# encryptorion-lab/phantom-fhe

Hardware: AMD Instinct MI355X
Metric: forward NTT limb-transforms/s at N=2^16, 45 RNS moduli (higher is better)
Workload: dtype u64; 1 GPU; CKKS N=2^16, 45 data limbs (+15 special), forward NTT of a batch of 16 ciphertext polynomials per step (720 limb-transforms, 360 MiB, HBM-resident; configs[2] parameter set); N=65536, limbs=45, special_limbs=15, parallelism=ciphertext-batch x1, launch=K steps enqueued by one library call (2 K eager kernel launches)

## Files before the change

### phantom-fhe_amd/csrc/pha_ntt.hip

```cpp
#include "../../include/phantom_amd.h"
#include "pha_internal.h"
#include "pha_experiments.h"
#include "pha_ntt_core.h"

#include <atomic>
#include <type_traits>

namespace pha {

constexpr int kPassHoist = 0;
#ifndef PHA_NTT_PASS_ORDER
#define PHA_NTT_PASS_ORDER 1
#endif
#ifndef PHA_NTT_ORDER_INT_HEAD
#define PHA_NTT_ORDER_INT_HEAD 1
#endif
#if defined(PHA_EXPERIMENTS)
std::atomic<int> g_ntt_variant{kDefaultVariant};
static inline int ntt_variant() { return g_ntt_variant.load(std::memory_order_relaxed); }
std::atomic<int> g_whole14_min{1 << 30};
std::atomic<int> g_fused_split{0};
std::atomic<int> g_fused_lag{2};
std::atomic<int> g_fused_min_tiles{1 << 30};
extern std::atomic<int> g_bconv_split;
// ... 41 lines not shown
template <bool FWD, int EPI, bool FOLD>
__device__ __forceinline__ void tile_args(const NttKArgs &k, uint32_t twr, uint32_t tile, PassArgs &a) {
    const uint32_t prime = twr >= k.sel.remap_from ? twr + k.sel.remap_add : twr;
    const size_t n = (size_t)1 << k.log_n;
    a.in = k.in + (size_t)twr * n;
    a.out = k.out + (size_t)twr * n;
    a.tw = k.tw + (size_t)prime * n;
    a.twd = nullptr;
    a.q = k.mod[prime].value;
    a.tile = tile;
    a.rho0 = k.t1;
    a.stride = k.t2;
    if (!FWD && FOLD) {
        a.ninv = k.ninv[prime];
        a.w1ninv = k.w1ninv[prime];
    }
    a.pro_reduce = false;
    a.pro_ratio1 = 0;
    a.fp = false;
    if (k.fpinfo) {
        const FpInfo fi = k.fpinfo[prime];
        if (fi.ok) {
            a.fp = true;
            a.fpm = FpMod{fi.q, fi.qinv, (fi.ok & 2) != 0, (fi.ok & 4) != 0};
            a.twd = k.twf + (size_t)prime * n;
            if (!FWD && FOLD) {
                a.ninv = k.ninvf[prime];
                a.w1ninv = k.w1ninvf[prime];
            }
        }
    }
    if (EPI == EPI_INV_SCALE || EPI == EPI_FWD_MODDOWN || EPI == EPI_FWD_MODDOWN_ADD || EPI == EPI_FWD_KSRESCALE) {
        a.scale.x = k.scale[twr];
        a.scale.y = k.scale_shoup[twr];
    }
    a.aux = (EPI == EPI_FWD_MODDOWN || EPI == EPI_FWD_MODDOWN_ADD || EPI == EPI_FWD_KSRESCALE || EPI == EPI_INV_CANON_ADD) ? k.aux + (size_t)twr * n : nullptr;
    if (EPI == EPI_FWD_KSRESCALE) {
        a.scale2.x = k.scale2[twr];
        a.scale2.y = k.scale2_shoup[twr];
        a.aux2 = k.aux2 + (size_t)twr * n;
    }
}

PHA_HD bool limb_excluded(const NttKArgs &k, uint32_t twr, uint32_t z) {
    const uint32_t zd = k.excl_mod ? z % k.excl_mod : z;
    const uint32_t es = k.sel.excl_start + zd * k.excl_step;
    uint32_t ee = es + (k.sel.excl_end - k.sel.excl_start);
    ee = ee < k.excl_limit ? ee : k.excl_limit;
    return twr >= es && twr < ee;
}

template <class C, bool FWD, int EPI, bool FOLD>
__device__ __forceinline__ void full_tile_args(const NttKArgs &k, uint32_t twr, uint32_t z, uint32_t tile, PassArgs &a) {
    tile_args<FWD, EPI, FOLD>(k, twr, tile, a);
    if (k.batch > 1) {
        a.in += (size_t)z * k.in_stride;
        a.out += (size_t)z * k.out_stride;
        if (EPI == EPI_FWD_MODDOWN || EPI == EPI_FWD_MODDOWN_ADD || EPI == EPI_FWD_KSRESCALE) a.aux += (size_t)z * k.aux_stride;
        if (EPI == EPI_FWD_KSRESCALE) a.aux2 += (size_t)z * k.aux2_stride;
    }
    if (EPI == EPI_INV_CANON_ADD) a.aux += (size_t)(z >> 1) * k.aux_pair_stride + (size_t)(z & 1) * k.aux_stride;
    if (FWD && (C::STRIDED || C::WHOLE) && k.pro_src) {
        const uint32_t prime = twr >= k.sel.remap_from ? twr + k.sel.remap_add : twr;
        a.in = k.pro_src + (size_t)z * k.pro_stride;
        a.pro_reduce = true;
        a.pro_ratio1 = k.mod[prime].ratio1;
        a.pro_half = bfv_lift_threshold(k.pro_t);
        a.pro_inc = bfv_lift_increment(a.q, k.pro_t);
    }
}

template <class C, bool FWD, int EPI, bool FOLD, int HOIST, bool COH, int ONLY = 0, int PRO = PRO_NONE>
__device__ __forceinline__ void exec_pass(const PassArgs &a, u64 *lds, int tid) {
    u64 reg[C::EPT];
    u64x2 twreg[C::TW_TOTAL];
    using Prog = PassProgram<C, FWD, EPI, FOLD, HOIST, COH, PRO>;
    auto pass = [&](const PassArgs &pa) __attribute__((always_inline)) {
        Prog::load_twiddles(pa, tid, twreg);
        Prog::template run_pass<SEG_PLAIN, false>(pa, lds, tid, reg, twreg);
    };
    PHA_WITH_FP_KNOWN(a, ONLY != 2 && a.fp, pass);
}

template <class C, bool FWD, int EPI, bool FOLD>
__global__ __launch_bounds__(C::THREADS) void ntt_zloop_kernel(const NttKArgs k, const ZloopMap m) {
    static_assert(!C::WHOLE, "the batched form exists for the passes of the two-pass plans");
    extern __shared__ __attribute__((aligned(16))) unsigned char smem[];
    u64 *lds = reinterpret_cast<u64 *>(smem);
    __builtin_amdgcn_s_setprio(3);
    const int tid = threadIdx.x;
    uint32_t b = blockIdx.x;
    PassArgs a;
    if (b < m.int_blocks) {
        const uint32_t tile = b % m.tiles, rest = b / m.tiles, z = rest % k.batch, twr = k.sel.start + m.limb[rest / k.batch];
        if (limb_excluded(k, twr, z)) return;
        full_tile_args<C, FWD, EPI, FOLD>(k, twr, z, tile, a);
        exec_pass<C, FWD, EPI, FOLD, 0, false, 2>(a, lds, tid);
        return;
    }
    b -= m.int_blocks;
    const uint32_t tile = b % m.tiles, rest = b / m.tiles, zgroups = (k.batch + m.zper - 1) / m.zper;
    const uint32_t twr = k.sel.start + m.limb[m.n_int + rest / zgroups];
    const uint32_t z0 = (rest % zgroups) * m.zper, z1 = (z0 + m.zper < k.batch) ? z0 + m.zper : k.batch;
    full_tile_args<C, FWD, EPI, FOLD>(k, twr, z0, tile, a);
    using Prog = PassProgram<C, FWD, EPI, FOLD, 1, false>;
    a.fp = true;
    u64x2 twreg[C::TW_TOTAL];
    Prog::load_twiddles(a, tid, twreg);
    u64 regA[C::EPT], regB[C::EPT];
    auto args_of = [&](uint32_t z) __attribute__((always_inline)) {
        PassArgs b = a;
        const size_t dz = (size_t)(z - z0);
        b.in += dz * k.in_stride;
        b.out += dz * k.out_stride;
        if (EPI == EPI_FWD_MODDOWN || EPI == EPI_FWD_MODDOWN_ADD || EPI == EPI_FWD_KSRESCALE) b.aux += dz * k.aux_stride;
        if (EPI == EPI_FWD_KSRESCALE) b.aux2 += dz * k.aux2_stride;
        return b;
    };
    auto transform = [&](const PassArgs &b, u64 *reg) __attribute__((always_inline)) {
        Prog::template run_pass<SEG_PREFETCHED, true>(b, lds, tid, reg, twreg);
    };
    auto next = [&](uint32_t z) __attribute__((always_inline)) {
        while (z < z1 && limb_excluded(k, twr, z)) z++;
        return z;
    };
    uint32_t z = next(z0);
    if (z >= z1) return;
    Prog::prefetch(args_of(z), tid, regA);
    __builtin_amdgcn_s_setprio(0);
    for (;;) {
        uint32_t zn = next(z + 1);
        if (zn < z1) Prog::prefetch(args_of(zn), tid, regB);
        transform(args_of(z), regA);
        if (zn >= z1) break;
        z = zn;
        zn = next(z + 1);
        if (zn < z1) Prog::prefetch(args_of(zn), tid, regA);
        transform(args_of(z), regB);
        if (zn >= z1) break;
        z = zn;
    }
}

template <class C, bool FWD, int EPI, bool FOLD, int HOIST, int PRO = PRO_NONE>
__global__ __launch_bounds__(C::THREADS) void ntt_pass_kernel(const NttKArgs k, const PassOrder o) {
    extern __shared__ __attribute__((aligned(16))) unsigned char smem[];
    u64 *lds = reinterpret_cast<u64 *>(smem);

    __builtin_amdgcn_s_setprio(3);
    uint32_t tile = blockIdx.x, y = blockIdx.y, z = blockIdx.z;
    if (k.zfast_tiles) {
        const uint32_t b = blockIdx.x, per_chunk = k.zfast_run * k.batch, chunk = b / per_chunk, rem = b - chunk * per_chunk;
        z = rem / k.zfast_run;
        const uint32_t group = chunk * k.zfast_run + (rem - z * k.zfast_run);
        if (group >= k.zfast_tiles * k.sel.count) return;
        tile = group % k.zfast_tiles;
        y = group / k.zfast_tiles;
    }
#if PHA_NTT_PASS_ORDER
    else if (o.tiles) {
        if (!pass_order_decode(o, k.batch, blockIdx.x, blockIdx.y, blockIdx.z, y, z, tile)) return;
    }
#endif
    const uint32_t twr = k.sel.start + y;
    if (limb_excluded(k, twr, z)) return;
    PassArgs a;
    full_tile_args<C, FWD, EPI, FOLD>(k, twr, z, tile, a);
    exec_pass<C, FWD, EPI, FOLD, HOIST, false, 0, PRO>(a, lds, threadIdx.x);
}

static void raise_lds_limit(const void *kernel, size_t bytes, std::atomic<uint64_t> &raised) {
    if (bytes <= 64 * 1024) return;
    int dev = 0;
    PHA_HIP(hipGetDevice(&dev));
    const uint64_t bit = 1ull << (dev & 63);
    if (raised.load(std::memory_order_acquire) & bit) return;
    PHA_HIP(hipFuncSetAttribute(kernel, hipFuncAttributeMaxDynamicSharedMemorySize, (int)bytes));
    raised.fetch_or(bit, std::memory_order_release);
}

template <class C, bool FWD, int EPI, bool FOLD, int PRO = PRO_NONE>
static void launch_pass(const NttKArgs &k, hipStream_t s, const PassOrder *order = nullptr) {
    const size_t n = (size_t)1 << k.log_n;
    const size_t lds_bytes = (size_t)C::LDS_WORDS * sizeof(u64);
    const unsigned tiles_per_limb = (unsigned)(n >> C::LOGTILE);
    dim3 grid(tiles_per_limb, k.sel.count, k.batch);
    NttKArgs kk = k;
    kk.zfast_tiles = 0;
    if (!C::STRIDED && !C::WHOLE && k.zfast_tiles) {
        kk.zfast_tiles = tiles_per_limb;
        kk.zfast_run = 8;
        const unsigned groups = tiles_per_limb * k.sel.count;
        grid = dim3(((groups + kk.zfast_run - 1) / kk.zfast_run) * kk.zfast_run * k.batch, 1, 1);
    }
    PassOrder o{};
    if (order && !kk.zfast_tiles) {
        o = *order;
        pass_order_grid(o, k.batch, grid.x, grid.y, grid.z);
    }
    static std::atomic<uint64_t> raised{0};
    raise_lds_limit(reinterpret_cast<const void *>(&ntt_pass_kernel<C, FWD, EPI, FOLD, kPassHoist, PRO>), lds_bytes, raised);
    hipLaunchKernelGGL((ntt_pass_kernel<C, FWD, EPI, FOLD, kPassHoist, PRO>), grid, dim3(C::THREADS), lds_bytes, s, kk, o);
    check_launch();
}

#if defined(PHA_EXPERIMENTS)
}
#include "pha_ntt_onelaunch.h"
namespace pha {
constexpr bool kExperiments = true;
#else
constexpr bool kExperiments = false;
#endif

template <int E> using EpiC = std::integral_constant<int, E>;
template <int P> using ProC = std::integral_constant<int, P>;
template <bool FWD, class F>
static void dispatch_epi(int epi, F &&f) {
    if constexpr (FWD) {
        if (epi == EPI_FWD_MODDOWN) f(EpiC<EPI_FWD_MODDOWN>{});
        else if (epi == EPI_FWD_MODDOWN_ADD) f(EpiC<EPI_FWD_MODDOWN_ADD>{});
        else if (epi == EPI_FWD_KSRESCALE) f(EpiC<EPI_FWD_KSRESCALE>{});
        else f(EpiC<EPI_FWD_CANON>{});
    } else {
        if (epi == EPI_INV_SCALE) f(EpiC<EPI_INV_SCALE>{});
        else if (epi == EPI_INV_CANON_ADD) f(EpiC<EPI_INV_CANON_ADD>{});
        else f(EpiC<EPI_INV_CANON>{});
    }
}
template <class F>
static void dispatch_pro(const NttKArgs &k, F &&f) {
    if (k.pro_t) f(ProC<PRO_LIFT>{});
    else f(ProC<PRO_NONE>{});
}

template <class P>
static void launch_inverse_last(const NttKArgs &k, int epi, hipStream_t s, const PassOrder *order = nullptr) {
    dispatch_epi<false>(epi, [&](auto e) { launch_pass<P, false, e(), true>(k, s, order); });
}

template <class W, bool FWD>
static void launch_whole(NttKArgs k, int epi, hipStream_t s) {
    k.t1 = 1;
    k.t2 = W::T;
    k.mid = k.out;
    if constexpr (FWD) {
        dispatch_epi<true>(epi, [&](auto e) {
            if constexpr (e() == EPI_FWD_CANON) dispatch_pro(k, [&](auto p) { launch_pass<W, true, EPI_FWD_CANON, false, p()>(k, s); });
            else launch_pass<W, true, e(), false>(k, s);
        });
    } else {
        launch_inverse_last<W>(k, epi, s);
    }
}

template <class C>
static bool plan_zloop(const NttKArgs &k, ZloopMap &m) {
    if (k.pro_src || k.sel.count > 128) return false;
    uint8_t fp[128];
    for (uint32_t y = 0; y < k.sel.count; y++) {
        const uint32_t twr = k.sel.start + y, prime = twr >= k.sel.remap_from ? twr + k.sel.remap_add : twr;
        fp[y] = k.fpinfo != nullptr && (k.h_primes[prime] >> 50) == 0;
    }
    return zloop_plan(m, k.sel.count, fp, k.batch, (uint32_t)(((size_t)1 << k.log_n) >> C::LOGTILE), C::THREADS / 64, kZloopMinBatch);
}
template <class C, bool FWD, int EPI, bool FOLD>
static void launch_zloop(const NttKArgs &k, const ZloopMap &m, hipStream_t s) {
    NttKArgs kk = k;
    kk.zfast_tiles = 0;
    const size_t lds_bytes = (size_t)C::LDS_WORDS * sizeof(u64);
    hipLaunchKernelGGL((ntt_zloop_kernel<C, FWD, EPI, FOLD>), dim3(zloop_blocks(m, k.batch)), dim3(C::THREADS), lds_bytes, s, kk, m);
    check_launch();
}
template <class C>
static void launch_zloop_forward(const NttKArgs &k, const ZloopMap &m, int epi, hipStream_t s) {
    dispatch_epi<true>(epi, [&](auto e) { launch_zloop<C, true, e(), false>(k, m, s); });
}

constexpr size_t kLastLevelCacheBytes = (size_t)256 << 20;
static NttKArgs limb_range(const NttKArgs &k, uint32_t lo, uint32_t cnt) {
    NttKArgs h = k;
    h.sel.start = k.sel.start + lo;
    h.sel.count = cnt;
    return h;
}
static uint32_t order_parts(const NttKArgs &k) {
    const size_t bytes = ((size_t)k.sel.count * k.batch << k.log_n) * sizeof(u64);
    return PHA_NTT_PASS_ORDER == 2 && k.sel.count >= 2 && bytes > kLastLevelCacheBytes ? 2u : 1u;
}

template <class F>
static void for_each_order_part(const NttKArgs &k, const ZloopMap &m, int strided_logtile, F &&pair) {
    if (PHA_NTT_PASS_ORDER == 0) return pair(0u, k.sel.count, m, (const PassOrder *)nullptr);
    const uint32_t parts = order_parts(k), cut = pass_order_half(k.sel.count);
    for (uint32_t h = 0; h < parts; h++) {
        const uint32_t lo = h * cut, hi = parts == 1 ? k.sel.count : h ? k.sel.count : cut;
        const ZloopMap mh = parts == 1 ? m : zloop_sub(m, lo, hi, k.batch);
        const PassOrder o = pass_order_reverse(mh, (uint32_t)(((size_t)1 << k.log_n) >> strided_logtile), PHA_NTT_ORDER_INT_HEAD != 0);
        pair(lo, hi - lo, mh, &o);
    }
}

constexpr int kIpPlan = 3;
template <int LOGN, int VARIANT>
struct TwoPass {
    using P1 = typename NttPlan<LOGN, VARIANT>::P1;
    using P2 = typename NttPlan<LOGN, VARIANT>::P2;
    static constexpr bool ZLOOP = zloop_variant(VARIANT) >= 0;
    using Z2 = typename NttPlan<LOGN, ZLOOP ? zloop_variant(VARIANT) : VARIANT>::P2;
    static constexpr bool ONE_LAUNCH = kExperiments && P1::THREADS == 512 && P1::LOGTILE == 12 && P2::THREADS == 64;
    NttKArgs k1, k2;
    explicit TwoPass(NttKArgs k) {
        k.t1 = P1::T;
        k.t2 = P2::T;
        k1 = k2 = k;
        k1.out = k.mid;
        k1.out_stride = k.poly_stride;
        k2.in = k.mid;
        k2.in_stride = k.poly_stride;
    }
};

template <int LOGN, int VARIANT>
static void forward_impl(const NttKArgs &k_in, int epi, hipStream_t s, Context *fused) {
    using T = TwoPass<LOGN, VARIANT>;
    using P1 = typename T::P1;
    using P2 = typename T::P2;
    T t(k_in);
    const NttKArgs &k1 = t.k1;
    NttKArgs &k = t.k2;
    k.pro_src = nullptr;
    if (k.first_pass_done && !(LOGN == 16 && VARIANT == 10 && P1::LOGT == 6))
        throw std::logic_error("ntt_forward: first_pass_done needs the 64 x 1024 plan the fused conversion wrote");
#if defined(PHA_EXPERIMENTS)
    if constexpr (T::ONE_LAUNCH) {
        if (fused && epi != EPI_FWD_KSRESCALE && !k.first_pass_done && !k.pro_t) {
            bool done = false;
            dispatch_epi<true>(epi, [&](auto e) {
                if constexpr (e() != EPI_FWD_KSRESCALE) done = launch_fused<P1, P2, true, e(), false>(*fused, k1, k, s);
            });
            if (done) return;
        }
    }
#endif
    auto strided = [&](const NttKArgs &ka, const PassOrder *order) {
        dispatch_pro(ka, [&](auto p) { launch_pass<P1, true, EPI_NONE, false, p()>(ka, s, order); });
    };
    if constexpr (T::ZLOOP) {
        using Z2 = typename T::Z2;
        ZloopMap m;
        if (!k.first_pass_only && plan_zloop<Z2>(k, m)) {
            if (k.first_pass_done) return launch_zloop_forward<Z2>(k, m, epi, s);
            return for_each_order_part(k, m, P1::LOGTILE, [&](uint32_t lo, uint32_t cnt, const ZloopMap &mh, const PassOrder *o) {
// ... 401 lines not shown
```

### phantom-fhe_amd/csrc/pha_ntt_core.h

```cpp
#pragma once
#include "pha_arith.h"
#include "pha_bfv_lift.h"

namespace pha {

constexpr int kTileElems = 4096;

enum Epilogue {
    EPI_NONE = 0,
    EPI_FWD_CANON = 1,
    EPI_FWD_MODDOWN = 2,
    EPI_INV_CANON = 3,
    EPI_INV_SCALE = 4,
    EPI_FWD_MODDOWN_ADD = 5,
    EPI_FWD_KSRESCALE = 6,
    EPI_INV_CANON_ADD = 7,
};

enum Prologue {
    PRO_NONE = 0,
    PRO_LIFT = 1,
};

template <int LOGT_, bool STRIDED_, int R0_, int R1_, int R2_ = 0, int EPT_ = 16, bool OT_ = false, int LOGTILE_ = 12,
          bool WHOLE_ = false, int R3_ = 0>
struct PassCfg {
    static constexpr int EPT = EPT_;
    static constexpr bool OT = OT_ && !STRIDED_;
    static constexpr int LOGTILE = LOGTILE_;
    static constexpr int TILE = 1 << LOGTILE_;
    static constexpr int THREADS = TILE / EPT_;
    static_assert(LOGTILE_ >= LOGT_ && LOGTILE_ <= 14, "a tile holds whole transforms and fits the LDS budget (2^14 words + padding = 144 KiB of the 160 KiB)");
    static constexpr bool WAVE_LOCAL = TILE / EPT_ == 64;
    static constexpr bool WHOLE = WHOLE_ && !STRIDED_;
    static_assert((1 << R0_) <= EPT_ && (1 << R1_) <= EPT_ && (1 << R2_) <= EPT_ && (1 << R3_) <= EPT_, "radix exceeds registers");
    static_assert(!R3_ || R2_, "rounds are filled in order");
    static constexpr int LOGT = LOGT_;
    static constexpr int T = 1 << LOGT_;
    static constexpr int LOGV = LOGTILE_ - LOGT_;
    static constexpr int V = 1 << LOGV;
    static constexpr bool STRIDED = STRIDED_;
    static constexpr int NR = R3_ ? 4 : R2_ ? 3 : 2;
    static_assert(R0_ + R1_ + R2_ + R3_ == LOGT_, "round schedule must cover all stages");
    static_assert(LOGT_ >= 4 && LOGT_ <= 14, "tile transform length out of range");
    static_assert(THREADS >= 64, "a workgroup is at least one wavefront");
    static constexpr int r(int i) { return i == 0 ? R0_ : i == 1 ? R1_ : i == 2 ? R2_ : R3_; }
    static constexpr bool ot_round(int i) { return OT && i == NR - 1; }
    static constexpr int tw_count(int i) {
        return !r(i) ? 0 : ot_round(i) ? ((1 << r(i)) - 1) + (EPT_ >> r(i)) * r(i) : (EPT_ >> r(i)) * ((1 << r(i)) - 1);
    }
    static constexpr int tw_off(int i) {
        return i == 0 ? 0 : i == 1 ? tw_count(0) : i == 2 ? tw_count(0) + tw_count(1) : tw_count(0) + tw_count(1) + tw_count(2);
    }
    static constexpr int TW_TOTAL = tw_count(0) + tw_count(1) + tw_count(2) + tw_count(3);
    static constexpr int s0(int i) { return i == 0 ? 0 : i == 1 ? R0_ : i == 2 ? R0_ + R1_ : R0_ + R1_ + R2_; }
    static constexpr int PITCH = T + ((T >> 4) << 1);
    static constexpr int LDS_WORDS = STRIDED_ ? (T * V + (T >> 4) * 16) : (V * PITCH);
    static constexpr int lds_index(int e, int v) {
        return STRIDED_ ? (e * V + v + ((e >> 4) << 4)) : (v * PITCH + e + ((e >> 4) << 1));
    }
};

struct PassArgs {
    const u64 *in;
    u64 *out;
    const u64x2 *tw;
    const u64 *twd;
    u64 q;
    u32 tile;
    u32 rho0;
    u32 stride;
    u64x2 ninv, w1ninv;
    u64x2 scale;
    const u64 *aux;
    u64x2 scale2;
    const u64 *aux2;
    bool fp;
    FpMod fpm;
    bool pro_reduce;
    u64 pro_ratio1;
    u64 pro_half, pro_inc;
};

template <class C>
PHA_HD size_t global_index(const PassArgs &a, int e, int v) {
    if (C::STRIDED) return (size_t)e * a.stride + (size_t)a.tile * C::V + v;
    return ((size_t)a.tile * C::V + v) * C::T + e;
}

template <class C, int RI>
PHA_HD void decode_group(int g, int &v, int &hi, int &lo) {
    constexpr int r = C::r(RI), s0 = C::s0(RI), LOGD = C::LOGT - s0 - r;
    if (C::STRIDED) {
        v = g & (C::V - 1);
        int rest = g >> C::LOGV;
        lo = rest & ((1 << LOGD) - 1);
        hi = rest >> LOGD;
    } else {
        lo = g & ((1 << LOGD) - 1);
        int rest = g >> LOGD;
        hi = rest & ((1 << s0) - 1);
        v = rest >> s0;
    }
}

PHA_HD u64x2 tw_entry(const PassArgs &a, u32 idx) {
    if (a.fp) return u64x2{a.twd[idx], 0};
    return a.tw[idx];
}
template <int R>
PHA_HD void load_group_twiddles(u64x2 *t, const PassArgs &a, u32 base0) {
    if (a.fp) {
#pragma unroll
        for (int j = 0; j < R; j++)
#pragma unroll
            for (int kk = 0; kk < (1 << j); kk++) t[(1 << j) - 1 + kk].x = a.twd[(base0 << j) + kk];
        return;
    }
#pragma unroll
    for (int j = 0; j < R; j++)
#pragma unroll
        for (int kk = 0; kk < (1 << j); kk++) t[(1 << j) - 1 + kk] = a.tw[(base0 << j) + kk];
}

template <int R>
PHA_HD void ct_round(u64 *v, const u64x2 *t, u64 q4, u64 nq) {
#pragma unroll
    for (int j = 0; j < R; j++) {
        const int dist = 1 << (R - 1 - j);
#pragma unroll
        for (int k = 0; k < (1 << R); k++) {
            if (k & dist) continue;
            const int kk = k >> (R - j);
            ct_bfly4(v[k], v[k + dist], t[(1 << j) - 1 + kk], q4, nq);
        }
    }
}

template <int R, bool FWD>
PHA_HD void ot_round_int(u64 *v, const u64x2 *tc, const u64x2 *tr, u64 q4, u64 nq) {
#pragma unroll
    for (int jj = 0; jj < R; jj++) {
        const int j = FWD ? jj : R - 1 - jj;
        const int dist = 1 << (R - 1 - j);
#pragma unroll
        for (int k = 0; k < (1 << R); k++) {
            if (k & dist) continue;
// ... 187 lines not shown
    return *p;
}
template <bool NT>
PHA_HD void gstore(u64 *p, u64 v) {
#if defined(__HIP_DEVICE_COMPILE__)
    if (NT) {
        __builtin_nontemporal_store(v, p);
        return;
    }
#endif
    *p = v;
}
template <bool NT>
PHA_HD void gstore2(u64x2 *p, u64x2 v) {
#if defined(__HIP_DEVICE_COMPILE__)
    if (NT) {
        __builtin_nontemporal_store(u64v2{v.x, v.y}, reinterpret_cast<u64v2 *>(p));
        return;
    }
#endif
    *p = v;
}

template <class C, int RI, bool FROM_GLOBAL, bool COH = false>
PHA_HD void round_load(const PassArgs &a, const u64 *lds, int tid, u64 *reg) {
    constexpr int r = C::r(RI), K = 1 << r, G = C::EPT >> r, s0 = C::s0(RI);
    constexpr int LOGD = C::LOGT - s0 - r;
#pragma unroll
    for (int gi = 0; gi < G; gi++) {
        int v, hi, lo;
        decode_group<C, RI>(tid + C::THREADS * gi, v, hi, lo);
        u64 *rg = reg + gi * K;
        const int e0 = (hi << (LOGD + r)) + lo;
        if (FROM_GLOBAL && COH) {
#if defined(__HIP_DEVICE_COMPILE__)
            if constexpr (!C::STRIDED && K == 8 && G == 1 && LOGD >= 1 && LOGD <= 6) {
                const bool odd = lo & 1;
                const u64 *base = a.in + global_index<C>(a, e0 - (odd ? 1 : 0) + ((odd ? 4 : 0) << LOGD), v);
                u64x2 w0, w1, w2, w3;
                asm volatile("global_load_dwordx4 %0, %4, off sc1\n\t"
                             "global_load_dwordx4 %1, %4, off offset:%5 sc1\n\t"
                             "global_load_dwordx4 %2, %4, off offset:%6 sc1\n\t"
                             "global_load_dwordx4 %3, %4, off offset:%7 sc1\n\t"
                             "s_waitcnt vmcnt(0)"
                             : "=&v"(w0), "=&v"(w1), "=&v"(w2), "=&v"(w3)
                             : "v"(base), "n"(8 << LOGD), "n"(16 << LOGD), "n"(24 << LOGD)
                             : "memory");
                const u64x2 w[4] = {w0, w1, w2, w3};
#pragma unroll
                for (int j = 0; j < 4; j++) {
                    const u64 send = odd ? w[j].x : w[j].y;
                    const u32 slo = (u32)__builtin_amdgcn_update_dpp(0, (int)(u32)send, 0xB1, 0xF, 0xF, false);
                    const u32 shi = (u32)__builtin_amdgcn_update_dpp(0, (int)(u32)(send >> 32), 0xB1, 0xF, 0xF, false);
                    const u64 recv = ((u64)shi << 32) | slo;
                    rg[j] = odd ? recv : w[j].x;
                    rg[4 + j] = odd ? w[j].y : recv;
                }
                continue;
            }
#endif
#pragma unroll
            for (int k = 0; k < K; k++) rg[k] = coherent_load(a.in + global_index<C>(a, e0 + (k << LOGD), v));
        } else if (FROM_GLOBAL) {
            if (!C::STRIDED && LOGD == 0) {
                const u64x2 *p = reinterpret_cast<const u64x2 *>(a.in + global_index<C>(a, e0, v));
#pragma unroll
                for (int k = 0; k < K; k += 2) {
                    u64x2 t = gload2<false>(p + (k >> 1));
                    rg[k] = t.x;
                    rg[k + 1] = t.y;
                }
            } else {
#pragma unroll
                for (int k = 0; k < K; k++) rg[k] = gload<false>(a.in + global_index<C>(a, e0 + (k << LOGD), v));
            }
        } else {
#pragma unroll
            for (int k = 0; k < K; k++) rg[k] = lds[C::lds_index(e0 + (k << LOGD), v)];
        }
    }
}

template <class C, int RI>
PHA_HD void round_load_tw(const PassArgs &a, int tid, u64x2 *twreg) {
    constexpr int r = C::r(RI), K = 1 << r, G = C::EPT >> r, s0 = C::s0(RI);
    if (C::ot_round(RI)) {
        static_assert(!C::ot_round(RI) || (C::THREADS % (1 << s0)) == 0, "groups of a thread must share hi");
        u64x2 *base = twreg + C::tw_off(RI);
        int v, hi, lo;
        decode_group<C, RI>(tid, v, hi, lo);
        load_group_twiddles<r>(base, a, (u32)hi);
#pragma unroll
        for (int gi = 0; gi < G; gi++) {
            decode_group<C, RI>(tid + C::THREADS * gi, v, hi, lo);
            const u32 rho = a.rho0 + a.tile * C::V + (u32)v;
#pragma unroll
            for (int j = 0; j < r; j++) base[(K - 1) + gi * r + j] = tw_entry(a, rho << (s0 + j));
        }
        return;
    }
#pragma unroll
    for (int gi = 0; gi < G; gi++) {
        int v, hi, lo;
        decode_group<C, RI>(tid + C::THREADS * gi, v, hi, lo);
        const u32 rho = C::STRIDED ? 1u : (a.rho0 + a.tile * C::V + (u32)v);
        const u32 base0 = (rho << s0) + (u32)hi;
        load_group_twiddles<r>(twreg + C::tw_off(RI) + gi * (K - 1), a, base0);
    }
}

template <class C, int RI, bool FWD, bool FOLD, bool RECENTRE = false, bool GSFULL = false>
PHA_HD void round_compute(const PassArgs &a, int tid, u64 *reg, const u64x2 *twreg) {
    constexpr int r = C::r(RI), K = 1 << r, G = C::EPT >> r;
    const u64 q4 = a.q << 2, nq = 0 - a.q;
    if (C::ot_round(RI)) {
        const u64x2 *tc = twreg + C::tw_off(RI);
#pragma unroll
        for (int gi = 0; gi < G; gi++) {
            u64 *rg = reg + gi * K;
            const u64x2 *tr = tc + (K - 1) + gi * r;
            if (a.fp) {
                if (FWD ? a.fpm.ct_light : a.fpm.gs_light) ot_round_fp<r, FWD, true>(rg, tc, tr, a.fpm);
                else ot_round_fp<r, FWD, false>(rg, tc, tr, a.fpm);
            } else {
                ot_round_int<r, FWD>(rg, tc, tr, q4, nq);
            }
        }
        return;
    }
    if (a.fp) {
#pragma unroll
        for (int gi = 0; gi < G; gi++) {
            u64 *rg = reg + gi * K;
            const u64x2 *t = twreg + C::tw_off(RI) + gi * (K - 1);
            if (FWD) {
                fp_ct_round<r>(rg, t, a.fpm);
                if (RECENTRE && !a.fpm.ct_light) {
#pragma unroll
                    for (int k = 0; k < K; k++) rg[k] = as_u64(fp_reduce(as_f64(rg[k]), a.fpm));
                }
            } else if (a.fpm.gs_light) {
                constexpr int stage0 = C::LOGT - C::s0(RI) - r;
                constexpr bool canon_in = !C::STRIDED;
                const bool light = C::LOGT <= 9 || a.fpm.q < (double)(1ull << (52 - C::LOGT));
                if (light) fp_gs_round<r, FOLD, true>(rg, t, a.fpm, a.ninv, a.w1ninv);
                else fp_gs_round<r, FOLD, false, stage0, canon_in>(rg, t, a.fpm, a.ninv, a.w1ninv);
            } else {
                if (GSFULL) {
                    constexpr bool canon = RI == C::NR - 1 && (!C::STRIDED || C::WHOLE);
                    fp_gs_round<r, FOLD, false, 0, canon>(rg, t, a.fpm, a.ninv, a.w1ninv);
                } else {
                    fp_gs_round<r, FOLD, true>(rg, t, a.fpm, a.ninv, a.w1ninv);
                }
                if (RECENTRE) {
#pragma unroll
                    for (int k = 0; k < K; k++) rg[k] = as_u64(fp_reduce(as_f64(rg[k]), a.fpm));
                }
            }
        }
        return;
    }
#pragma unroll
    for (int gi = 0; gi < G; gi++) {
        u64 *rg = reg + gi * K;
        const u64x2 *t = twreg + C::tw_off(RI) + gi * (K - 1);
        if (FWD) ct_round<r>(rg, t, q4, nq);
        else gs_round<r, FOLD>(rg, t, q4, nq, a.ninv, a.w1ninv);
    }
}

template <class C, int RI, bool TO_GLOBAL, int EPI>
PHA_HD void round_out(const PassArgs &a, u64 *lds, int tid, const u64 *reg) {
    constexpr int r = C::r(RI), K = 1 << r, G = C::EPT >> r, s0 = C::s0(RI);
    constexpr int LOGD = C::LOGT - s0 - r;
#pragma unroll
    for (int gi = 0; gi < G; gi++) {
        int v, hi, lo;
        decode_group<C, RI>(tid + C::THREADS * gi, v, hi, lo);
        const u64 *rg = reg + gi * K;
        const int e0 = (hi << (LOGD + r)) + lo;
        if (TO_GLOBAL) {
            if (!C::STRIDED && LOGD == 0) {
                const size_t g0 = global_index<C>(a, e0, v);
                u64x2 *p = reinterpret_cast<u64x2 *>(a.out + g0);
#pragma unroll
                for (int k = 0; k < K; k += 2) {
                    u64x2 aux{0, 0}, acc{0, 0};
                    if (EPI == EPI_FWD_MODDOWN || EPI == EPI_FWD_MODDOWN_ADD || EPI == EPI_FWD_KSRESCALE || EPI == EPI_INV_CANON_ADD)
                        aux = reinterpret_cast<const u64x2 *>(a.aux + g0)[k >> 1];
                    if (EPI == EPI_FWD_MODDOWN_ADD) acc = p[k >> 1];
                    if (EPI == EPI_FWD_KSRESCALE) acc = reinterpret_cast<const u64x2 *>(a.aux2 + g0)[k >> 1];
                    u64x2 t;
                    t.x = apply_epilogue_v<EPI>(rg[k], a, aux.x, acc.x);
                    t.y = apply_epilogue_v<EPI>(rg[k + 1], a, aux.y, acc.y);
                    gstore2<false>(p + (k >> 1), t);
                }
            } else {
#pragma unroll
                for (int k = 0; k < K; k++) {
                    const size_t gidx = global_index<C>(a, e0 + (k << LOGD), v);
                    gstore<false>(a.out + gidx, apply_epilogue<EPI>(rg[k], a, gidx));
                }
            }
        } else {
#pragma unroll
            for (int k = 0; k < K; k++) lds[C::lds_index(e0 + (k << LOGD), v)] = rg[k];
        }
    }
}

template <class C>
PHA_HD void tile_sync() {
#if defined(__HIP_DEVICE_COMPILE__)
    if constexpr (C::WAVE_LOCAL) {
        __builtin_amdgcn_fence(__ATOMIC_RELEASE, "wavefront");
        __builtin_amdgcn_wave_barrier();
        __builtin_amdgcn_fence(__ATOMIC_ACQUIRE, "wavefront");
    } else {
        __syncthreads();
    }
#endif
}

enum SegMode { SEG_PLAIN = 0, SEG_PREFETCHED = 1, SEG_KEEP = 2 };

template <class C, bool FWD, int EPI, bool FOLD, int HOIST = 1, bool COH = false, int PRO = PRO_NONE>
struct PassProgram {
    static constexpr int NSEG = C::NR;
    static constexpr int THREADS = C::THREADS;
    static constexpr bool FIRST_PASS = C::WHOLE || (FWD ? C::STRIDED : !C::STRIDED);
    static constexpr bool LAST_PASS = C::WHOLE || !(FWD ? C::STRIDED : !C::STRIDED);

    static constexpr double kFpLimit = 7.5;
    struct FpSched {
        bool recentre[4];
        bool full[4];
        double after[4];
    };
    static constexpr double fp_grow(double m, int stages, bool full) {
        if (!FWD) {
            if (full) return 2.0;
            for (int i = 0; i < stages; i++) m = 2.0 * m + 1e-6;
            return m;
        }
        for (int i = 0; i < stages; i++) m = full ? m + 0.5 + 1e-6 : 1.375 * m + 0.5 + 1e-6;
        return m;
    }
    static constexpr FpSched fp_sched() {
        FpSched sc{};
        double m = FIRST_PASS ? 1.0 : 0.5 + 1e-6;
        for (int seg = 0; seg < C::NR; seg++) {
            const int ri = FWD ? seg : C::NR - 1 - seg;
            sc.full[seg] = !FWD && !C::ot_round(ri) && fp_grow(m, C::r(ri), false) > kFpLimit;
            m = fp_grow(m, C::r(ri), C::ot_round(ri) || sc.full[seg]);
            sc.after[seg] = m;
            bool rc = false;
            if (seg == C::NR - 1) rc = !LAST_PASS;
            else {
                const int rn = FWD ? seg + 1 : C::NR - 2 - seg;
                rc = fp_grow(m, C::r(rn), C::ot_round(rn)) > kFpLimit;
            }
            sc.recentre[seg] = rc;
            if (rc) m = 0.5 + 1e-6;
        }
        return sc;
    }
    static constexpr bool fp_sched_ok() {
        const FpSched sc = fp_sched();
        for (int seg = 0; seg < C::NR; seg++) {
            if (sc.after[seg] > kFpLimit) return false;
            const int ri = FWD ? seg : C::NR - 1 - seg;
            if (C::ot_round(ri) && (sc.full[seg] || (FWD && sc.recentre[seg]))) return false;
        }
        return true;
    }
    static_assert(fp_sched_ok(), "FP64 path: a round would take the registers past 7.5 q (exactness needs < 8 q at 50 bits), or the schedule asks an on-the-fly-twiddle round to re-centre");

    PHA_HD static void fp_after_global_load(const PassArgs &a, u64 *reg) {
        if (!a.fp) return;
        if (!FIRST_PASS && !(FWD ? a.fpm.ct_light : a.fpm.gs_light)) return;
#pragma unroll
        for (int i = 0; i < C::EPT; i++)
            reg[i] = as_u64(FIRST_PASS ? fp_from_canon(reg[i]) : fp_reduce(as_f64(reg[i]), a.fpm));
    }
    PHA_HD static void fp_before_global_store(const PassArgs &a, u64 *reg) {
        if (!a.fp || !LAST_PASS) return;
        if (fp_epilogue(EPI)) return;
#pragma unroll
        for (int i = 0; i < C::EPT; i++) reg[i] = fp_to_canon(as_f64(reg[i]), a.fpm);
    }

    static constexpr int round_of(int seg) { return FWD ? seg : C::NR - 1 - seg; }
    PHA_HD static void load_twiddles(const PassArgs &a, int tid, u64x2 *twreg) {
        if (HOIST == 1) {
            round_load_tw<C, 0>(a, tid, twreg);
            round_load_tw<C, 1>(a, tid, twreg);
            if (C::NR >= 3) round_load_tw<C, 2>(a, tid, twreg);
            if (C::NR == 4) round_load_tw<C, 3>(a, tid, twreg);
        } else if (HOIST == 2) {
            round_load_tw<C, round_of(0)>(a, tid, twreg);
        }
    }
    template <int SEG>
    PHA_HD static void segment_twiddles(const PassArgs &a, int tid, u64x2 *twreg) {
        if (HOIST == 0) round_load_tw<C, round_of(SEG)>(a, tid, twreg);
        if (HOIST == 2 && SEG + 1 < C::NR) round_load_tw<C, round_of(SEG + 1 < C::NR ? SEG + 1 : SEG)>(a, tid, twreg);
    }

    template <int SEG, int MODE>
    PHA_HD static void segment(const PassArgs &a, u64 *lds, int tid, u64 *reg, u64x2 *twreg) {
        constexpr int RI = round_of(SEG);
        constexpr bool first = SEG == 0, last = SEG == C::NR - 1;
        static_assert(MODE != SEG_KEEP || (last && !first), "the kept segment is the last one of a multi-round pass");
        static_assert(MODE != SEG_KEEP || !(fp_sched().recentre[SEG] || fp_sched().full[SEG]), "a kept segment hands over what the rounds left");
        segment_twiddles<SEG>(a, tid, twreg);
        if constexpr (!(first && MODE == SEG_PREFETCHED)) round_load<C, RI, first, COH>(a, lds, tid, reg);
        if constexpr (first && MODE == SEG_PLAIN) {
#if defined(__HIP_DEVICE_COMPILE__)
            __builtin_amdgcn_s_setprio(0);
#endif
            if constexpr (PRO == PRO_LIFT) {
                static_assert(FWD && FIRST_PASS, "the plain lift is the load prologue of a forward transform's first pass");
#pragma unroll
                for (int i = 0; i < C::EPT; i++) reg[i] = bfv_lift_word(reg[i], a.pro_half, a.pro_inc);
            } else if (FWD && FIRST_PASS && a.pro_reduce) {
#pragma unroll
                for (int i = 0; i < C::EPT; i++) reg[i] = barrett64(reg[i], a.q, a.pro_ratio1);
            }
        }
        static_assert(PRO != PRO_LIFT || MODE == SEG_PLAIN, "the load prologue belongs to the pass that loads");
        if (first) fp_after_global_load(a, reg);
        if (FWD && C::WHOLE && C::LOGT >= 14 && SEG == 2 && a.fp) {
#pragma unroll
            for (int i = 0; i < C::EPT; i++) reg[i] = as_u64(fp_reduce(as_f64(reg[i]), a.fpm));
        }
        round_compute<C, RI, FWD, FOLD && RI == 0, fp_sched().recentre[SEG], fp_sched().full[SEG]>(a, tid, reg, twreg);
        if constexpr (MODE != SEG_KEEP) {
            if (last) fp_before_global_store(a, reg);
            round_out<C, RI, last, last ? EPI : (int)EPI_NONE>(a, lds, tid, reg);
        }
    }
    template <int SEG>
    PHA_HD static void run(const PassArgs &a, u64 *lds, int tid, u64 *reg, u64x2 *twreg) { segment<SEG, SEG_PLAIN>(a, lds, tid, reg, twreg); }
    template <int SEG>
    PHA_HD static void run_prefetched(const PassArgs &a, u64 *lds, int tid, u64 *reg, u64x2 *twreg) { segment<SEG, SEG_PREFETCHED>(a, lds, tid, reg, twreg); }
    template <int SEG>
    PHA_HD static void run_keep(const PassArgs &a, u64 *lds, int tid, u64 *reg, u64x2 *twreg) { segment<SEG, SEG_KEEP>(a, lds, tid, reg, twreg); }

    PHA_HD static void prefetch(const PassArgs &a, int tid, u64 *reg) { round_load<C, round_of(0), true>(a, nullptr, tid, reg); }

    template <int MODE, bool TAIL_SYNC, int SEG = 0>
    PHA_HD static void run_pass(const PassArgs &a, u64 *lds, int tid, u64 *reg, u64x2 *twreg) {
        constexpr bool last = SEG == NSEG - 1;
        segment<SEG, (MODE == SEG_KEEP && !last) ? (int)SEG_PLAIN : MODE>(a, lds, tid, reg, twreg);
        if constexpr (!last) {
            tile_sync<C>();
            run_pass<MODE, TAIL_SYNC, SEG + 1>(a, lds, tid, reg, twreg);
        } else if constexpr (TAIL_SYNC) {
            tile_sync<C>();
        }
    }
};

#define PHA_WITH_FP_KNOWN(a, cond, body) \
    if (cond) {                          \
        PassArgs b_ = (a);               \
        b_.fp = true;                    \
        body(b_);                        \
    } else {                             \
        PassArgs b_ = (a);               \
        b_.fp = false;                   \
        body(b_);                        \
    }

template <int LOGN, int VARIANT> struct NttPlan;
template <> struct NttPlan<12, 0> { using P1 = PassCfg<6, true, 3, 3>;  using P2 = PassCfg<6, false, 3, 3>; };
template <> struct NttPlan<13, 0> { using P1 = PassCfg<6, true, 3, 3>;  using P2 = PassCfg<7, false, 4, 3>; };
template <> struct NttPlan<14, 0> { using P1 = PassCfg<7, true, 4, 3>;  using P2 = PassCfg<7, false, 4, 3>; };
template <> struct NttPlan<15, 0> { using P1 = PassCfg<7, true, 4, 3>;  using P2 = PassCfg<8, false, 4, 4>; };
template <> struct NttPlan<16, 0> { using P1 = PassCfg<8, true, 4, 4>;  using P2 = PassCfg<8, false, 4, 4>; };
template <> struct NttPlan<17, 0> { using P1 = PassCfg<8, true, 4, 4>;  using P2 = PassCfg<9, false, 3, 3, 3>; };
template <> struct NttPlan<12, 1> { using P1 = PassCfg<6, true, 3, 3, 0, 8>;  using P2 = PassCfg<6, false, 3, 3, 0, 8>; };
template <> struct NttPlan<13, 1> { using P1 = PassCfg<6, true, 3, 3, 0, 8>;  using P2 = PassCfg<7, false, 3, 2, 2, 8>; };
template <> struct NttPlan<14, 1> { using P1 = PassCfg<7, true, 3, 2, 2, 8>;  using P2 = PassCfg<7, false, 3, 2, 2, 8>; };
template <> struct NttPlan<15, 1> { using P1 = PassCfg<7, true, 3, 2, 2, 8>;  using P2 = PassCfg<8, false, 3, 3, 2, 8>; };
template <> struct NttPlan<16, 1> { using P1 = PassCfg<8, true, 3, 3, 2, 8>;  using P2 = PassCfg<8, false, 3, 3, 2, 8>; };
template <> struct NttPlan<17, 1> { using P1 = PassCfg<8, true, 3, 3, 2, 8>;  using P2 = PassCfg<9, false, 3, 3, 3, 8>; };
template <> struct NttPlan<12, 2> { using P1 = PassCfg<6, true, 3, 3, 0, 8>;  using P2 = PassCfg<6, false, 3, 3, 0, 8, true>; };
template <> struct NttPlan<13, 2> { using P1 = PassCfg<6, true, 3, 3, 0, 8>;  using P2 = PassCfg<7, false, 3, 2, 2, 8, true>; };
template <> struct NttPlan<14, 2> { using P1 = PassCfg<7, true, 3, 2, 2, 8>;  using P2 = PassCfg<7, false, 3, 2, 2, 8, true>; };
template <> struct NttPlan<15, 2> { using P1 = PassCfg<7, true, 3, 2, 2, 8>;  using P2 = PassCfg<8, false, 3, 3, 2, 8, true>; };
template <> struct NttPlan<16, 2> { using P1 = PassCfg<8, true, 3, 3, 2, 8>;  using P2 = PassCfg<8, false, 3, 3, 2, 8, true>; };
template <> struct NttPlan<17, 2> { using P1 = PassCfg<8, true, 3, 3, 2, 8>;  using P2 = PassCfg<9, false, 3, 3, 3, 8, true>; };
template <> struct NttPlan<12, 3> { using P1 = PassCfg<6, true, 3, 3, 0, 8>;  using P2 = PassCfg<6, false, 3, 3, 0, 8, false, 9>; };
template <> struct NttPlan<13, 3> { using P1 = PassCfg<6, true, 3, 3, 0, 8>;  using P2 = PassCfg<7, false, 3, 2, 2, 8, false, 9>; };
template <> struct NttPlan<14, 3> { using P1 = PassCfg<7, true, 3, 2, 2, 8>;  using P2 = PassCfg<7, false, 3, 2, 2, 8, false, 9>; };
template <> struct NttPlan<15, 3> { using P1 = PassCfg<7, true, 3, 2, 2, 8>;  using P2 = PassCfg<8, false, 3, 3, 2, 8, false, 9>; };
template <> struct NttPlan<16, 3> { using P1 = PassCfg<8, true, 3, 3, 2, 8>;  using P2 = PassCfg<8, false, 3, 3, 2, 8, false, 9>; };
template <> struct NttPlan<17, 3> { using P1 = PassCfg<8, true, 3, 3, 2, 8>;  using P2 = PassCfg<9, false, 3, 3, 3, 8, false, 9>; };
template <> struct NttPlan<12, 4> { using P1 = PassCfg<6, true, 3, 3, 0, 8>;  using P2 = PassCfg<6, false, 3, 3, 0, 8, true, 9>; };
template <> struct NttPlan<13, 4> { using P1 = PassCfg<6, true, 3, 3, 0, 8>;  using P2 = PassCfg<7, false, 3, 2, 2, 8, true, 9>; };
template <> struct NttPlan<14, 4> { using P1 = PassCfg<7, true, 3, 2, 2, 8>;  using P2 = PassCfg<7, false, 3, 2, 2, 8, true, 9>; };
template <> struct NttPlan<15, 4> { using P1 = PassCfg<7, true, 3, 2, 2, 8>;  using P2 = PassCfg<8, false, 3, 3, 2, 8, true, 9>; };
template <> struct NttPlan<16, 4> { using P1 = PassCfg<8, true, 3, 3, 2, 8>;  using P2 = PassCfg<8, false, 3, 3, 2, 8, true, 9>; };
template <> struct NttPlan<17, 4> { using P1 = PassCfg<8, true, 3, 3, 2, 8>;  using P2 = PassCfg<9, false, 3, 3, 3, 8, true, 9>; };
template <> struct NttPlan<14, 5> { using P1 = PassCfg<7, true, 3, 2, 2, 8>;  using P2 = PassCfg<7, false, 2, 2, 2, 4, false, 8, false, 1>; };
template <> struct NttPlan<15, 5> { using P1 = PassCfg<7, true, 3, 2, 2, 8>;  using P2 = PassCfg<8, false, 2, 2, 2, 4, false, 8, false, 2>; };
template <> struct NttPlan<16, 5> { using P1 = PassCfg<8, true, 3, 3, 2, 8>;  using P2 = PassCfg<8, false, 2, 2, 2, 4, false, 8, false, 2>; };
template <> struct NttPlan<14, 6> { using P1 = PassCfg<7, true, 2, 2, 2, 4, false, 11, false, 1>;  using P2 = NttPlan<14, 5>::P2; };
template <> struct NttPlan<15, 6> { using P1 = PassCfg<7, true, 2, 2, 2, 4, false, 11, false, 1>;  using P2 = NttPlan<15, 5>::P2; };
template <> struct NttPlan<16, 6> { using P1 = PassCfg<8, true, 2, 2, 2, 4, false, 11, false, 2>;  using P2 = NttPlan<16, 5>::P2; };
template <> struct NttPlan<14, 7> { using P1 = PassCfg<7, true, 2, 2, 2, 4, false, 12, false, 1>;  using P2 = NttPlan<14, 5>::P2; };
template <> struct NttPlan<15, 7> { using P1 = PassCfg<7, true, 2, 2, 2, 4, false, 12, false, 1>;  using P2 = NttPlan<15, 5>::P2; };
template <> struct NttPlan<16, 7> { using P1 = PassCfg<8, true, 2, 2, 2, 4, false, 12, false, 2>;  using P2 = NttPlan<16, 5>::P2; };
template <> struct NttPlan<16, 8> { using P1 = PassCfg<7, true, 3, 2, 2, 8>;  using P2 = PassCfg<9, false, 3, 3, 3, 8, false, 9>; };
template <> struct NttPlan<16, 9> { using P1 = PassCfg<7, true, 3, 2, 2, 8>;  using P2 = PassCfg<9, false, 3, 3, 3, 8, true, 9>; };
template <> struct NttPlan<16, 10> { using P1 = PassCfg<6, true, 3, 3, 0, 8, false, 11>;  using P2 = PassCfg<10, false, 3, 3, 2, 8, false, 10, false, 2>; };
template <> struct NttPlan<16, 12> { using P1 = PassCfg<6, true, 3, 3, 0, 8>;  using P2 = PassCfg<10, false, 4, 3, 3, 16, false, 10>; };
template <> struct NttPlan<16, 13> { using P1 = PassCfg<6, true, 2, 2, 2, 4, false, 10>;  using P2 = NttPlan<16, 10>::P2; };
using WholePlan12 = PassCfg<12, false, 4, 4, 4, 16, false, 12, true>;
using WholePlan13 = PassCfg<13, false, 4, 4, 4, 16, false, 13, true, 1>;
using WholePlan14 = PassCfg<14, false, 4, 4, 4, 16, false, 14, true, 2>;

struct ZloopMap {
    uint32_t n_int, n_fp;
    uint32_t zper;
    uint32_t tiles;
    uint32_t int_blocks;
    uint8_t limb[128];
};

inline uint32_t zloop_zper(uint32_t batch, size_t wgs_per_poly, uint32_t waves_per_wg, uint32_t min_batch) {
// ... 126 lines not shown
```

Before: 2.790 million NTT/s.

## Stage next batch tile into LDS via global_load_lds in z-loop NTT kernel

For z-loop passes whose epilogues are simple, replaces register double-buffered prefetch (regA/regB) with asynchronous global_load_lds_dwordx4 copies of the next polynomial's tile into an extra LDS staging area, read back through a permutation map. This frees the second register buffer and overlaps the next tile's HBM load with the current transform. In exchange it uses an extra tile of LDS per block, which can reduce occupancy, and relies on inline asm with vmcnt accounting that must match the store count.

Result: faster. 2.831 million NTT/s (median of 6 runs) (+1.5%).

```diff
diff --git a/phantom-fhe_amd/csrc/pha_ntt.hip b/phantom-fhe_amd/csrc/pha_ntt.hip
--- a/phantom-fhe_amd/csrc/pha_ntt.hip
+++ b/phantom-fhe_amd/csrc/pha_ntt.hip
@@ -147,6 +147,10 @@
     PHA_WITH_FP_KNOWN(a, ONLY != 2 && a.fp, pass);
 }
 
+template <class C>
+constexpr bool zloop_staged(int epi) {
+    return !C::WAVE_LOCAL && (epi == EPI_NONE || epi == EPI_FWD_CANON || epi == EPI_INV_CANON || epi == EPI_INV_SCALE);
+}
 template <class C, bool FWD, int EPI, bool FOLD>
 __global__ __launch_bounds__(C::THREADS) void ntt_zloop_kernel(const NttKArgs k, const ZloopMap m) {
     static_assert(!C::WHOLE, "the batched form exists for the passes of the two-pass plans");
@@ -172,7 +176,6 @@
     a.fp = true;
     u64x2 twreg[C::TW_TOTAL];
     Prog::load_twiddles(a, tid, twreg);
-    u64 regA[C::EPT], regB[C::EPT];
     auto args_of = [&](uint32_t z) __attribute__((always_inline)) {
         PassArgs b = a;
         const size_t dz = (size_t)(z - z0);
@@ -182,15 +185,32 @@
         if (EPI == EPI_FWD_KSRESCALE) b.aux2 += dz * k.aux2_stride;
         return b;
     };
-    auto transform = [&](const PassArgs &b, u64 *reg) __attribute__((always_inline)) {
-        Prog::template run_pass<SEG_PREFETCHED, true>(b, lds, tid, reg, twreg);
-    };
     auto next = [&](uint32_t z) __attribute__((always_inline)) {
         while (z < z1 && limb_excluded(k, twr, z)) z++;
         return z;
     };
     uint32_t z = next(z0);
     if (z >= z1) return;
+    if constexpr (zloop_staged<C>(EPI)) {
+        u64 reg[C::EPT];
+        Prog::stage_first(args_of(z), lds, tid);
+        __builtin_amdgcn_s_setprio(0);
+        stage_wait<0>();
+        for (;;) {
+            const uint32_t zn = next(z + 1);
+            PassArgs b = args_of(z);
+            b.in_next = zn < z1 ? args_of(zn).in : nullptr;
+            Prog::template run_pass<SEG_STAGED, true>(b, lds, tid, reg, twreg);
+            if (zn >= z1) break;
+            stage_wait<Prog::TILE_STORES>();
+            z = zn;
+        }
+        return;
+    }
+    u64 regA[C::EPT], regB[C::EPT];
+    auto transform = [&](const PassArgs &b, u64 *reg) __attribute__((always_inline)) {
+        Prog::template run_pass<SEG_PREFETCHED, true>(b, lds, tid, reg, twreg);
+    };
     Prog::prefetch(args_of(z), tid, regA);
     __builtin_amdgcn_s_setprio(0);
     for (;;) {
@@ -333,7 +353,7 @@
 static void launch_zloop(const NttKArgs &k, const ZloopMap &m, hipStream_t s) {
     NttKArgs kk = k;
     kk.zfast_tiles = 0;
-    const size_t lds_bytes = (size_t)C::LDS_WORDS * sizeof(u64);
+    const size_t lds_bytes = (size_t)(zloop_staged<C>(EPI) ? C::LDS_WORDS + C::TILE : C::LDS_WORDS) * sizeof(u64);
     hipLaunchKernelGGL((ntt_zloop_kernel<C, FWD, EPI, FOLD>), dim3(zloop_blocks(m, k.batch)), dim3(C::THREADS), lds_bytes, s, kk, m);
     check_launch();
 }
diff --git a/phantom-fhe_amd/csrc/pha_ntt_core.h b/phantom-fhe_amd/csrc/pha_ntt_core.h
--- a/phantom-fhe_amd/csrc/pha_ntt_core.h
+++ b/phantom-fhe_amd/csrc/pha_ntt_core.h
@@ -63,6 +63,7 @@
 
 struct PassArgs {
     const u64 *in;
+    const u64 *in_next;
     u64 *out;
     const u64x2 *tw;
     const u64 *twd;
@@ -416,6 +417,65 @@
 }
 
 template <class C, int RI>
+struct StageMap {
+    static_assert(!C::STRIDED, "the staging row holds whole rows of a contiguous pass");
+    static constexpr int LOGD = C::LOGT - C::s0(RI) - C::r(RI);
+    static constexpr unsigned WAVES = C::THREADS / 64, WAVE_WORDS = 64 * C::EPT, WORDS = C::TILE, REQUESTS = C::EPT / 2;
+    static constexpr unsigned RUN = WAVES == 1 ? WORDS : LOGD == 0 ? (64u << C::r(RI)) : (LOGD >= 6 && (1u << (LOGD - 6)) >= WAVES) ? 64u : 0u;
+    static_assert(RUN != 0, "the words a wavefront reads in this round are not aligned runs that alternate between the wavefronts");
+    PHA_HD static constexpr unsigned image_of(unsigned t) { return ((t / RUN) % WAVES) * WAVE_WORDS + (t / (RUN * WAVES)) * RUN + t % RUN; }
+    PHA_HD static constexpr unsigned word_of(unsigned p) { return ((p % WAVE_WORDS) / RUN) * (RUN * WAVES) + (p / WAVE_WORDS) * RUN + p % RUN; }
+    PHA_HD static constexpr unsigned request_image(unsigned wave, unsigned i, unsigned lane) { return wave * WAVE_WORDS + i * 128 + 2 * lane; }
+    static constexpr bool consistent() {
+        for (unsigned t = 0; t < WORDS; t++)
+            if (image_of(t) >= WORDS || word_of(image_of(t)) != t) return false;
+        return RUN % 2 == 0 && WAVE_WORDS % RUN == 0;
+    }
+};
+
+template <class C, int RI>
+PHA_HD void round_load_staged(const u64 *stage, int tid, u64 *reg) {
+    using M = StageMap<C, RI>;
+    static_assert(M::consistent(), "image_of / word_of are not inverse permutations of the tile");
+    constexpr int r = C::r(RI), K = 1 << r, G = C::EPT >> r, LOGD = M::LOGD;
+#pragma unroll
+    for (int gi = 0; gi < G; gi++) {
+        int v, hi, lo;
+        decode_group<C, RI>(tid + C::THREADS * gi, v, hi, lo);
+        const unsigned t0 = (unsigned)(v * C::T + (hi << (LOGD + r)) + lo);
+#pragma unroll
+        for (int k = 0; k < K; k++) reg[gi * K + k] = stage[M::image_of(t0 + ((unsigned)k << LOGD))];
+    }
+}
+
+template <class C, int RI>
+PHA_HD void stage_request(const PassArgs &a, const u64 *in, u64 *stage, int tid) {
+#if defined(__HIP_DEVICE_COMPILE__)
+    using M = StageMap<C, RI>;
+    const unsigned lane = (unsigned)tid & 63u, wave = (unsigned)tid >> 6;
+    const u64 *src = in + global_index<C>(a, 0, 0);
+    const unsigned dst = (unsigned)__builtin_amdgcn_readfirstlane(
+        (int)(unsigned)(uintptr_t)(__attribute__((address_space(3))) u64 *)(stage + wave * M::WAVE_WORDS));
+    asm volatile("s_waitcnt lgkmcnt(0)" ::: "memory");
+#pragma unroll
+    for (unsigned i = 0; i < M::REQUESTS; i++) {
+        const u64 *g = src + M::word_of(M::request_image(wave, i, lane));
+        unsigned keep;
+        asm volatile("s_mov_b32 %0, m0\n\ts_mov_b32 m0, %2\n\ts_nop 0\n\tglobal_load_lds_dwordx4 %1, off\n\ts_mov_b32 m0, %0"
+                     : "=&s"(keep)
+                     : "v"(g), "s"(dst + i * 1024u)
+                     : "memory");
+    }
+#endif
+}
+template <int STILL>
+PHA_HD void stage_wait() {
+#if defined(__HIP_DEVICE_COMPILE__)
+    asm volatile("s_waitcnt vmcnt(%0)" ::"n"(STILL) : "memory");
+#endif
+}
+
+template <class C, int RI>
 PHA_HD void round_load_tw(const PassArgs &a, int tid, u64x2 *twreg) {
     constexpr int r = C::r(RI), K = 1 << r, G = C::EPT >> r, s0 = C::s0(RI);
     if (C::ot_round(RI)) {
@@ -556,7 +616,7 @@
 #endif
 }
 
-enum SegMode { SEG_PLAIN = 0, SEG_PREFETCHED = 1, SEG_KEEP = 2 };
+enum SegMode { SEG_PLAIN = 0, SEG_PREFETCHED = 1, SEG_KEEP = 2, SEG_STAGED = 3 };
 
 template <class C, bool FWD, int EPI, bool FOLD, int HOIST = 1, bool COH = false, int PRO = PRO_NONE>
 struct PassProgram {
@@ -648,7 +708,13 @@
         static_assert(MODE != SEG_KEEP || (last && !first), "the kept segment is the last one of a multi-round pass");
         static_assert(MODE != SEG_KEEP || !(fp_sched().recentre[SEG] || fp_sched().full[SEG]), "a kept segment hands over what the rounds left");
         segment_twiddles<SEG>(a, tid, twreg);
-        if constexpr (!(first && MODE == SEG_PREFETCHED)) round_load<C, RI, first, COH>(a, lds, tid, reg);
+        if constexpr (first && MODE == SEG_STAGED) {
+            u64 *stage = lds + C::LDS_WORDS;
+            round_load_staged<C, RI>(stage, tid, reg);
+            if (a.in_next) stage_request<C, RI>(a, a.in_next, stage, tid);
+        } else if constexpr (!(first && MODE == SEG_PREFETCHED)) {
+            round_load<C, RI, first, COH>(a, lds, tid, reg);
+        }
         if constexpr (first && MODE == SEG_PLAIN) {
 #if defined(__HIP_DEVICE_COMPILE__)
             __builtin_amdgcn_s_setprio(0);
@@ -681,7 +747,13 @@
     template <int SEG>
     PHA_HD static void run_keep(const PassArgs &a, u64 *lds, int tid, u64 *reg, u64x2 *twreg) { segment<SEG, SEG_KEEP>(a, lds, tid, reg, twreg); }
 
+    template <int SEG>
+    PHA_HD static void run_staged(const PassArgs &a, u64 *lds, int tid, u64 *reg, u64x2 *twreg) { segment<SEG, SEG_STAGED>(a, lds, tid, reg, twreg); }
+
     PHA_HD static void prefetch(const PassArgs &a, int tid, u64 *reg) { round_load<C, round_of(0), true>(a, nullptr, tid, reg); }
+    using Stage = StageMap<C, round_of(0)>;
+    static constexpr int TILE_STORES = (C::LOGT - C::s0(round_of(C::NR - 1)) - C::r(round_of(C::NR - 1)) == 0) ? C::EPT / 2 : C::EPT;
+    PHA_HD static void stage_first(const PassArgs &a, u64 *lds, int tid) { stage_request<C, round_of(0)>(a, a.in, lds + C::LDS_WORDS, tid); }
 
     template <int MODE, bool TAIL_SYNC, int SEG = 0>
     PHA_HD static void run_pass(const PassArgs &a, u64 *lds, int tid, u64 *reg, u64x2 *twreg) {
```
